# acids-ircam/RAVE

Hardware: AMD Instinct MI355X
Metric: audio samples/sec/GPU (RAVE v2 training step, 44.1 kHz, n_signal=65536) (higher is better)
Workload: dtype f32; 1 GPU; v2 config, batch 32 mono 44.1 kHz n_signal=65536, VAE-phase training step per GPU (--phase vae); global_batch=32, parallelism=dp1, phase=vae

## Files before the change

rave_amd/csrc/conv_wgrad_x6.hip:

```cpp
#include <cstdlib>
#include <mutex>
#include <type_traits>
#include "conv_params.hpp"

namespace {

typedef unsigned u32x4 __attribute__((ext_vector_type(4)));
constexpr unsigned kOOB = 0x80000000u;

struct Wx6P {
    const float* R;
    const float* S;
    float* out;
    float* rsum;
    int B, M, C, T, N;
    int r_row, s_row, s_valid, is;
    float r_slope, s_slope;
    int steps_per_b;
    int total_steps, steps_per_z;
    unsigned r_bytes, s_bytes;
    int minoff, maxoff;
    int p8, cpb, chmax;
    int av;
    unsigned b_stage;
    const unsigned* r_range;
    const unsigned* s_range;
    int off[kMaxTaps];
};

typedef u32x4 u32x4_u __attribute__((aligned(2)));

__device__ __forceinline__ void emit(const float (&v)[8], float slope, float sc, u32x4* dst, int piece_stride) {
#if RH_X6_F16
    u32x4 hi, lo;
#pragma unroll
    for (int k = 0; k < 4; ++k) {
        float a = v[2 * k] * sc, b = v[2 * k + 1] * sc;
        a = rh_max1(a, a * slope);
        b = rh_max1(b, b * slope);
        const rh_h2 h = rh_h2_split(a, b);
        hi[k] = h.hi; lo[k] = h.lo;
    }
    dst[0] = hi;
    dst[piece_stride] = lo;
#else
    unsigned h[3][8];
#pragma unroll
    for (int i = 0; i < 8; ++i) {
        const float x = rh_max1(v[i], v[i] * slope);
        rh_bf3_split(x, h[0][i], h[1][i], h[2][i]);
    }
#pragma unroll
    for (int s3 = 0; s3 < 3; ++s3) {
        u32x4 pk;
#pragma unroll
        for (int k = 0; k < 4; ++k) pk[k] = __builtin_amdgcn_perm(h[s3][2 * k + 1], h[s3][2 * k], 0x07060302u);
        dst[s3 * piece_stride] = pk;
    }
#endif
}

constexpr int kKS = 2;
constexpr int kOct = 2 * kKS;
constexpr int kSpan = 16 * kKS;

constexpr int wx6_gs(int rows) { return kX6P * rows + 4; }
constexpr int wx6_stage(int rows) { return kKS * 2 * wx6_gs(rows); }
constexpr int wx6_slot(int o, int row, int rows) { return (o >> 1) * 2 * wx6_gs(rows) + (o & 1) * wx6_gs(rows) + row; }

struct Wx6Scale { float r, s, out; };
__device__ __forceinline__ Wx6Scale wx6_scales(const Wx6P& p) {
#if RH_X6_F16
    int inv_r, inv_s;
    Wx6Scale sc;
    sc.r = __uint_as_float(rh_x6_scale_bits(rh_range_max(p.r_range), &inv_r));
    sc.s = __uint_as_float(rh_x6_scale_bits(rh_range_max(p.s_range), &inv_s));
    sc.out = __uint_as_float(rh_x6_unscale_bits(inv_r, inv_s));
    return sc;
#else
    return Wx6Scale{1.f, 1.f, 1.f};
#endif
}

struct Wx6Step {
    int n;
    unsigned rs, ss;
    bool r_tail, s_edge;
};
template <bool PL>
__device__ __forceinline__ Wx6Step wx6_step(const Wx6P& p, int st) {
    Wx6Step sp;
    const int b = st / p.steps_per_b;
    sp.n = (st - b * p.steps_per_b) * kSpan;
    sp.rs = (unsigned)((b * p.M * p.r_row + sp.n) * 4);
    sp.ss = (unsigned)((b * p.C * p.s_row + sp.n * p.is) * 4);
    sp.r_tail = sp.n + kSpan > p.r_row;
    sp.s_edge = PL ? (sp.n + p.minoff < 0 || sp.n + p.minoff + 8 * p.p8 > p.s_valid || sp.r_tail)
                   : (sp.n * p.is + p.minoff < 0 || (sp.n + kSpan - 1) * p.is + p.maxoff >= p.s_valid || sp.r_tail);
    return sp;
}

template <int NT, int BM>
struct Wx6RTasks {
    static constexpr int NA = (kOct * BM + NT - 1) / NT;
    unsigned off[NA];
    int dst[NA], pos[NA];
    float v[NA][8];
    float sum[NA];

    __device__ __forceinline__ void init(const Wx6P& p, int tid, int m0) {
#pragma unroll
        for (int q = 0; q < NA; ++q) {
            const int u = tid + NT * q;
            const int o = u % kOct, m = u / kOct;
            const bool ok = m < BM && m0 + m < p.M;
            dst[q] = m < BM ? wx6_slot(o, m, BM) : -1;
            pos[q] = 8 * o;
            off[q] = ok ? (unsigned)(((m0 + m) * p.r_row + 8 * o) * 4) : kOOB;
            sum[q] = 0.f;
#pragma unroll
            for (int i = 0; i < 8; ++i) v[q][i] = 0.f;
        }
    }
    template <class RSRC>
    __device__ __forceinline__ void load(const Wx6P& p, RSRC rsrc, const Wx6Step& sp, bool av) {
#pragma unroll
        for (int q = 0; q < NA; ++q) {
            const unsigned base = off[q] == kOOB ? kOOB : off[q] + sp.rs;
            if (av) {
#pragma unroll
                for (int h = 0; h < 2; ++h) {
                    unsigned o = base == kOOB ? kOOB : base + 16u * h;
                    if (sp.r_tail) o = sp.n + pos[q] + 4 * h < p.r_row ? o : kOOB;
                    const u32x4 x = __builtin_bit_cast(u32x4, __builtin_amdgcn_raw_buffer_load_b128(rsrc, o, 0, 0));
#pragma unroll
                    for (int i = 0; i < 4; ++i) v[q][4 * h + i] = __uint_as_float(x[i]);
                }
            } else {
#pragma unroll
                for (int i = 0; i < 8; ++i) {
                    unsigned o = base == kOOB ? kOOB : base + 4u * i;
                    if (sp.r_tail) o = sp.n + pos[q] + i < p.r_row ? o : kOOB;
                    v[q][i] = __builtin_bit_cast(float, __builtin_amdgcn_raw_buffer_load_b32(rsrc, o, 0, 0));
                }
            }
        }
    }
    __device__ __forceinline__ void add_rows() {
#pragma unroll
        for (int q = 0; q < NA; ++q)
            sum[q] += ((v[q][0] + v[q][1]) + (v[q][2] + v[q][3])) + ((v[q][4] + v[q][5]) + (v[q][6] + v[q][7]));
    }
    __device__ __forceinline__ void store_sums(const Wx6P& p, int tid, int m0, int z) const {
#pragma unroll
        for (int q = 0; q < NA; ++q) {
            float s = sum[q];
            s += __shfl_xor(s, 1, 64);
            s += __shfl_xor(s, 2, 64);
            const int u = tid + NT * q;
            const int m = u / kOct;
            if ((u % kOct) == 0 && m < BM && m0 + m < p.M) p.rsum[(long)z * p.M + m0 + m] = s;
        }
    }
    __device__ __forceinline__ void convert(const Wx6P& p, float sc, u32x4* a_stage) const {
#pragma unroll
        for (int q = 0; q < NA; ++q)
            if (dst[q] >= 0) emit(v[q], p.r_slope, sc, a_stage + dst[q], BM);
    }
};

template <int NT, int NB, int BN, bool PL>
struct Wx6STasks {
    static_assert(PL || NT * NB == kOct * BN, "the (column, octet) tasks fill NB whole rounds");
    unsigned off[NB];
    int dst[NB], p0[NB];
    float v[NB][8];
    int c_lo;
    unsigned piece;

    __device__ __forceinline__ void init(const Wx6P& p, int first, int n0, bool part) {
        c_lo = PL ? n0 / p.T : 0;
        const int n_ch = PL ? min(p.N - 1, n0 + BN - 1) / p.T - c_lo + 1 : 0;
        piece = PL ? (unsigned)(p.chmax * p.cpb) : 16u * BN;
#pragma unroll
        for (int q = 0; q < NB; ++q) {
            const int u = first + NT * q;
            if constexpr (PL) {
                const int ch = u / p.p8, o = u - ch * p.p8;
                const bool ok = ch < n_ch;
                dst[q] = ok ? ch * p.cpb + o * 16 : -1;
                p0[q] = p.minoff + 8 * o;
                off[q] = ok ? (unsigned)(((c_lo + ch) * p.s_row + p0[q]) * 4) : kOOB;
            } else {
                const int o = u % kOct, col = u / kOct;
                const int cc = (n0 + col) / p.T, t = (n0 + col) - cc * p.T;
                const bool ok = n0 + col < p.N;
                dst[q] = (ok || !part) ? wx6_slot(o, col, BN) * 16 : -1;
                p0[q] = 8 * o * p.is + (ok ? p.off[t] : 0);
                off[q] = ok ? (unsigned)((cc * p.s_row + p0[q]) * 4) : kOOB;
            }
        }
    }
    __device__ __forceinline__ unsigned column(const Wx6P& p, int n, int tn) const {
        if constexpr (PL) {
            if (n >= p.N) return 0u;
            const int cc = n / p.T, t = n - cc * p.T;
            return (unsigned)((cc - c_lo) * p.cpb + (p.off[t] - p.minoff) * 2);
        } else {
            return 16u * 32u * tn;
        }
    }
    __device__ __forceinline__ static int kblock(int kb, int g, int colj) {
        return PL ? (kb * 16 + g * 8) * 2 : (kb * 2 * wx6_gs(BN) + g * wx6_gs(BN) + colj) * 16;
    }
    template <class RSRC>
    __device__ __forceinline__ void load(const Wx6P& p, RSRC rsrc, const Wx6Step& sp, int nq) {
#pragma unroll
        for (int q = 0; q < NB; ++q) {
            if (q >= nq) continue;
            const unsigned base = off[q] == kOOB ? kOOB : off[q] + sp.ss;
#pragma unroll
            for (int i = 0; i < 8; ++i) {
                unsigned o = base == kOOB ? kOOB : base + 4u * (unsigned)(i * p.is);
                if (sp.s_edge) {
                    const int pos = sp.n * p.is + p0[q] + i * p.is;
                    o = (pos >= 0 && pos < p.s_valid) ? o : kOOB;
                }
                v[q][i] = __builtin_bit_cast(float, __builtin_amdgcn_raw_buffer_load_b32(rsrc, o, 0, 0));
            }
        }
    }
    __device__ __forceinline__ void convert(const Wx6P& p, float sc, unsigned char* b_stage, int nq) const {
#pragma unroll
        for (int q = 0; q < NB; ++q) {
            if (q >= nq || dst[q] < 0) continue;
            emit(v[q], p.s_slope, sc, reinterpret_cast<u32x4*>(b_stage + dst[q]), (int)(piece >> 4));
        }
    }
};

template <int TM, int TN, int BM, bool PL>
__device__ __forceinline__ void wx6_mma(f32x16 (&acc)[TM][TN], const u32x4* al, const unsigned char* bl, const unsigned (&bcol)[TN],
                                        unsigned piece, bool live2) {
    constexpr int SA[RH_X6_NPROD] = RH_X6_SA, SB[RH_X6_NPROD] = RH_X6_SB;
    rh_x6_frag afr[TM][kX6P], bfr[TN][kX6P];
#pragma unroll
    for (int tm = 0; tm < TM; ++tm)
#pragma unroll
        for (int s3 = 0; s3 < kX6P; ++s3) afr[tm][s3] = __builtin_bit_cast(rh_x6_frag, al[s3 * BM + tm * 32]);
#pragma unroll
    for (int tn = 0; tn < TN; ++tn)
#pragma unroll
        for (int s3 = 0; s3 < kX6P; ++s3) {
            const unsigned char* f = bl + bcol[tn] + (unsigned)s3 * piece;
            if constexpr (PL) bfr[tn][s3] = __builtin_bit_cast(rh_x6_frag, *reinterpret_cast<const u32x4_u*>(f));
            else bfr[tn][s3] = __builtin_bit_cast(rh_x6_frag, *reinterpret_cast<const u32x4*>(f));
        }
#pragma unroll
    for (int q = 0; q < RH_X6_NPROD; ++q)
#pragma unroll
        for (int tm = 0; tm < TM; ++tm) {
            acc[tm][0] = RH_X6_MFMA(afr[tm][SA[q]], bfr[0][SB[q]], acc[tm][0]);
            if constexpr (TN == 2) {
                if (live2) acc[tm][1] = RH_X6_MFMA(afr[tm][SA[q]], bfr[1][SB[q]], acc[tm][1]);
            }
        }
}

__device__ __forceinline__ void wx6_store_tile(const Wx6P& p, float* __restrict__ outz, const f32x16& acc, int mb, int col, float osc) {
#pragma unroll
    for (int r = 0; r < 16; ++r) {
        const int m = mb + (r & 3) + 8 * (r >> 2);
        if (m < p.M) outz[(long)m * p.N + col] = RH_X6_F16 ? acc[r] * osc : acc[r];
    }
}

template <int TM, int WM, int WN, bool AV, bool PART, bool PL>
__global__ __launch_bounds__(256, 2) void wgrad_x6_kernel(const Wx6P p) {
    static_assert(WM * WN == 4, "four waves");
    constexpr int NT = 256, BM = 32 * TM * WM, BN = 64 * WN;
    constexpr int NB = PL ? ((BN / 2 + 2) * 7 + NT - 1) / NT : kOct * BN / NT;
    extern __shared__ __attribute__((aligned(16))) unsigned char smem_raw[];
    u32x4* const a_st = reinterpret_cast<u32x4*>(smem_raw);
    unsigned char* const b_st = smem_raw + wx6_stage(BM) * 16;

    const int tid = threadIdx.x, lane = tid & 63;
    const int wave = __builtin_amdgcn_readfirstlane(tid >> 6);
    const int j = lane & 31, g = lane >> 5;
    const int wm = wave / WN, wn = wave - wm * WN;
    const int m0 = blockIdx.y * BM, n0 = blockIdx.x * BN, z = blockIdx.z;

    const auto r_rsrc = __builtin_amdgcn_make_buffer_rsrc(const_cast<float*>(p.R), 0, p.r_bytes, 0x00020000);
    const auto s_rsrc = __builtin_amdgcn_make_buffer_rsrc(const_cast<float*>(p.S), 0, p.s_bytes, 0x00020000);
    const Wx6Scale sc = wx6_scales(p);

    Wx6RTasks<NT, BM> rt;
    Wx6STasks<NT, NB, BN, PL> stk;
    rt.init(p, tid, m0);
    stk.init(p, tid, n0, PART);
    unsigned bcol[2];
#pragma unroll
    for (int tn = 0; tn < 2; ++tn) bcol[tn] = stk.column(p, n0 + wn * 64 + tn * 32 + j, tn);

    f32x16 acc[TM][2];
#pragma unroll
    for (int tm = 0; tm < TM; ++tm)
#pragma unroll
        for (int tn = 0; tn < 2; ++tn)
#pragma unroll
            for (int r = 0; r < 16; ++r) acc[tm][tn][r] = 0.f;

    const bool want_rsum = p.rsum != nullptr && blockIdx.x == 0;
    auto load = [&](int st) {
        const Wx6Step sp = wx6_step<PL>(p, st);
        rt.load(p, r_rsrc, sp, AV);
        stk.load(p, s_rsrc, sp, NB);
    };
    auto convert = [&]() {
        if (want_rsum) rt.add_rows();
        rt.convert(p, sc.r, a_st);
        stk.convert(p, sc.s, b_st, NB);
    };

    const int st0 = z * p.steps_per_z;
    const int nst = min(p.steps_per_z, p.total_steps - st0);
    if (nst > 0) {
        load(st0);
        convert();
    }
    __syncthreads();
    const u32x4* const al = a_st + g * wx6_gs(BM) + wm * TM * 32 + j;
    const int live_tn = !PART ? 2 : (n0 + wn * 64 >= p.N ? 0 : (n0 + wn * 64 + 32 >= p.N ? 1 : 2));
    const bool live1 = live_tn >= 1, live2 = live_tn == 2;
    for (int s = 0; s < nst; ++s) {
        const bool more = s + 1 < nst;
        if (more) load(st0 + s + 1);
        if (live1) {
#pragma unroll
            for (int kb = 0; kb < kKS; ++kb)
                wx6_mma<TM, 2, BM, PL>(acc, al + kb * 2 * wx6_gs(BM), b_st + stk.kblock(kb, g, wn * 64 + j), bcol, stk.piece, live2);
        }
        __syncthreads();
        if (more) convert();
        __syncthreads();
    }

    if (want_rsum) rt.store_sums(p, tid, m0, z);
    float* __restrict__ outz = p.out + (long)z * p.M * p.N;
#pragma unroll
    for (int tn = 0; tn < 2; ++tn) {
        const int col = n0 + wn * 64 + tn * 32 + j;
        if (col >= p.N) continue;
#pragma unroll
        for (int tm = 0; tm < TM; ++tm) wx6_store_tile(p, outz, acc[tm][tn], m0 + (wm * TM + tm) * 32 + 4 * g, col, sc.out);
    }
}

template <int NW, bool PL>
__global__ __launch_bounds__(64 * NW) void wgrad_x6_wide_kernel(const Wx6P p) {
    constexpr int TM = 3, BM = 32 * TM, BN = 32 * NW, NT = 64 * NW;
    constexpr int NB = 2;
    extern __shared__ __attribute__((aligned(16))) unsigned char smem_raw[];
    u32x4* const a_st = reinterpret_cast<u32x4*>(smem_raw);
    unsigned char* const b_st = smem_raw + 2 * wx6_stage(BM) * 16;

    const int tid = threadIdx.x, lane = tid & 63;
    const int wave = __builtin_amdgcn_readfirstlane(tid >> 6);
    const int j = lane & 31, g = lane >> 5;
    const int z = blockIdx.x;

    const auto r_rsrc = __builtin_amdgcn_make_buffer_rsrc(const_cast<float*>(p.R), 0, p.r_bytes, 0x00020000);
    const auto s_rsrc = __builtin_amdgcn_make_buffer_rsrc(const_cast<float*>(p.S), 0, p.s_bytes, 0x00020000);
    const Wx6Scale sc = wx6_scales(p);

    Wx6RTasks<NT, BM> rt;
    Wx6STasks<NT, NB, BN, PL> stk;
    rt.init(p, tid, 0);
    stk.init(p, NT - 1 - tid, 0, true);
    const int nq = PL ? (p.C * p.p8 + NT - 1) / NT : NB;
    const bool r_wave = !(NT > kOct * BM && 64 * wave >= kOct * BM);
    const int col = 32 * wave + j;
    const bool live = 32 * wave < p.N;
    const unsigned bcol[1] = {stk.column(p, col, 0)};

    f32x16 acc[TM][1];
#pragma unroll
    for (int tm = 0; tm < TM; ++tm)
#pragma unroll
        for (int r = 0; r < 16; ++r) acc[tm][0][r] = 0.f;

    const bool want_rsum = p.rsum != nullptr;
    auto load = [&](int st) {
        const Wx6Step sp = wx6_step<PL>(p, st);
        if (r_wave) rt.load(p, r_rsrc, sp, p.av != 0);
        stk.load(p, s_rsrc, sp, nq);
    };
    auto convert = [&](int stage) {
        if (want_rsum) rt.add_rows();
        rt.convert(p, sc.r, a_st + stage * wx6_stage(BM));
        stk.convert(p, sc.s, b_st + stage * p.b_stage, nq);
    };
    auto multiply = [&](int stage) {
        const u32x4* const al = a_st + stage * wx6_stage(BM) + g * wx6_gs(BM) + j;
        const unsigned char* const bs = b_st + stage * p.b_stage;
#pragma unroll
        for (int kb = 0; kb < kKS; ++kb)
            wx6_mma<TM, 1, BM, PL>(acc, al + kb * 2 * wx6_gs(BM), bs + stk.kblock(kb, g, col), bcol, stk.piece, false);
    };

    const int st0 = z * p.steps_per_z;
    const int nst = min(p.steps_per_z, p.total_steps - st0);
    if (nst > 0) {
        load(st0);
        convert(0);
    }
    __syncthreads();
    for (int s = 0; s < nst; ++s) {
        const bool more = s + 1 < nst;
        if (more) load(st0 + s + 1);
        if (live) multiply(s & 1);
        if (more) convert((s + 1) & 1);
        __syncthreads();
    }

    if (want_rsum) rt.store_sums(p, tid, 0, z);
    if (col < p.N) {
        float* __restrict__ outz = p.out + (long)z * p.M * p.N;
#pragma unroll
        for (int tm = 0; tm < TM; ++tm) wx6_store_tile(p, outz, acc[tm][0], tm * 32 + 4 * g, col, sc.out);
    }
}

struct Wx6Plan {
    int tm, wm, rt, ct, Z, steps_per_z;
    int planes;
    int nw;
    int own_z;
    size_t lds;
};

struct Wx6Env {
    bool off;
    int planes;
    int wide;
    int blocks;
    int all;
    int tm;
    bool forced_tm() const { return tm >= 1 && tm <= 3; }
};

Wx6Env read_wx6_env() {
    const auto num = [](const char* name, int dflt) { const char* e = getenv(name); return e ? atoi(e) : dflt; };
    static const int all = num("RH_WGRAD_X6_ALL", 0), tm = num("RH_WGRAD_X6_TM", 0);
    const char* pe = getenv("RH_WGRAD_X6_PLANES");
    return Wx6Env{num("RH_WGRAD_X6", 1) == 0, pe ? (pe[0] == '1' ? 1 : 0) : -1, num("RH_WGRAD_X6_WIDE", 1), num("RH_WGRAD_X6_BLOCKS", 0), all, tm};
}

bool wx6_eligible(const WgradP& w, const Wx6Env& env, const unsigned* r_range, const unsigned* s_range) {
    if (env.off) return false;
    if (RH_X6_F16 && (!r_range || !s_range)) return false;
    if (w.inner != 1 || w.T > kMaxTaps || w.B <= 0 || w.r_row <= 0) return false;
    if ((w.r_act != RH_ACT_NONE && w.r_act != RH_ACT_LEAKY) || (w.s_act != RH_ACT_NONE && w.s_act != RH_ACT_LEAKY)) return false;
    if ((w.r_act == RH_ACT_LEAKY && !(w.r_slope >= 0.f && w.r_slope <= 1.f)) || (w.s_act == RH_ACT_LEAKY && !(w.s_slope >= 0.f && w.s_slope <= 1.f))) return false;
    if (w.M < 32 || (long)w.C * w.T < 64) return false;
    if (!env.all && w.M <= 64 && w.r_row > 1024) return false;
    return 4ull * w.B * w.M * (unsigned long long)w.r_row < 0x7fffffffull && 4ull * w.B * w.C * (unsigned long long)w.s_row < 0x7fffffffull;
}

bool wx6_plane_geometry(const WgradP& w, int chmax, Wx6P* p, size_t* bytes) {
    const int reach = w.maxoff - w.minoff;
    p->p8 = (32 + reach + 7) / 8;
    p->cpb = 16 * ((p->p8 & 1) ? p->p8 : p->p8 + 1);
    p->chmax = chmax;
    *bytes = (size_t)kX6P * chmax * p->cpb + 32;
    return w.is == 1 && w.T >= 2 && reach >= 0 && p->p8 <= 7 && 4l * (w.s_row + 64) * w.C * w.B < 0x7fffffffl;
}

int wx6_choose_tile(const WgradP& w, const Wx6Env& env, Wx6P* p, Wx6Plan* pl) {
    const int Mp = (w.M + 31) & ~31;
    pl->tm = (Mp % 128 == 0 && Mp >= 256 && w.T > 1) ? 2 : (Mp % 96 == 0 ? 3 : (Mp % 64 == 0 ? 2 : 1));
    if (env.forced_tm()) pl->tm = env.tm;
    pl->wm = Mp >= 64 * pl->tm ? 2 : 1;
    const int BM = 32 * pl->tm * pl->wm, BN = 64 * (4 / pl->wm);
    pl->rt = rh_cdiv(w.M, BM);
    pl->ct = rh_cdiv(p->N, BN);
    const int four_wave_tiles = pl->rt * pl->ct;
    pl->nw = 0; pl->own_z = 0;
    size_t plane_bytes;
    if (env.wide != 0 && env.planes < 0 && !env.forced_tm() && w.M > 64 && w.M <= 96 && p->N <= 288) {
        const int tiles = rh_cdiv(p->N, 32);
        pl->nw = tiles <= 3 ? 3 : (tiles <= 4 ? 4 : (tiles <= 6 ? 6 : 9));
        pl->own_z = env.wide != 2;
        pl->tm = 3; pl->wm = 1; pl->rt = 1; pl->ct = 1;
        pl->planes = wx6_plane_geometry(w, w.C, p, &plane_bytes);
        p->av = w.r_row % 4 == 0 && ((uintptr_t)w.R & 15) == 0;
        p->b_stage = (unsigned)(pl->planes ? (plane_bytes + 15) / 16 * 16 : (size_t)wx6_stage(32 * pl->nw) * 16);
        pl->lds = 2 * ((size_t)wx6_stage(96) * 16 + p->b_stage);
    } else {
        const bool on = env.planes >= 0 ? env.planes == 1 : Mp <= 96;
        pl->planes = wx6_plane_geometry(w, BN / w.T + 2, p, &plane_bytes) && on && pl->tm >= 2;
        pl->lds = (size_t)wx6_stage(BM) * 16 + (pl->planes ? plane_bytes : (size_t)wx6_stage(BN) * 16);
    }
    return four_wave_tiles;
}

void wx6_slice_k(const Wx6Env& env, int four_wave_tiles, Wx6P* p, Wx6Plan* pl) {
    const int dflt = pl->nw == 9 && pl->own_z ? 256 : 512;
    const int target = env.blocks > 0 ? env.blocks : (env.blocks < 0 ? (pl->tm == 2 ? 768 : 512) : dflt);
    int Z = rh_cdiv(target, pl->own_z ? 1 : four_wave_tiles);
    const int zmax = p->total_steps / 4 > 0 ? p->total_steps / 4 : 1;
    if (Z > zmax) Z = zmax;
    if (Z < 1) Z = 1;
    pl->steps_per_z = rh_cdiv(p->total_steps, Z);
    pl->Z = rh_cdiv(p->total_steps, pl->steps_per_z);
    p->steps_per_z = pl->steps_per_z;
}

bool plan_wx6(const WgradP& w, Wx6P* p, Wx6Plan* pl, const unsigned* r_range, const unsigned* s_range) {
    const Wx6Env env = read_wx6_env();
    if (!wx6_eligible(w, env, r_range, s_range)) return false;
    *p = Wx6P{};
    p->R = w.R; p->S = w.S;
    p->B = w.B; p->M = w.M; p->C = w.C; p->T = w.T; p->N = w.C * w.T;
    p->r_row = w.r_row; p->s_row = w.s_row; p->s_valid = w.s_valid; p->is = w.is;
    p->r_slope = w.r_act == RH_ACT_LEAKY ? w.r_slope : 1.f;
    p->s_slope = w.s_act == RH_ACT_LEAKY ? w.s_slope : 1.f;
    p->steps_per_b = rh_cdiv(w.r_row, kSpan);
    p->total_steps = w.B * p->steps_per_b;
    p->r_bytes = (unsigned)(4ull * w.B * w.M * w.r_row); p->s_bytes = (unsigned)(4ull * w.B * w.C * w.s_row);
    p->minoff = w.minoff; p->maxoff = w.maxoff;
    p->r_range = r_range; p->s_range = s_range;
    for (int t = 0; t < w.T; ++t) p->off[t] = w.off[t];
    wx6_slice_k(env, wx6_choose_tile(w, env, p, pl), p, pl);
    return true;
}

using Wx6Launch = void (*)(dim3 grid, int threads, size_t lds, hipStream_t stream, const Wx6P& p);

template <void (*KERN)(Wx6P)>
void launch_wx6(dim3 grid, int threads, size_t lds, hipStream_t stream, const Wx6P& p) {
    static std::once_flag once;
    std::call_once(once, [] {
        (void)hipFuncSetAttribute(reinterpret_cast<const void*>(KERN), hipFuncAttributeMaxDynamicSharedMemorySize, 160 * 1024);
    });
    rh_launch_main(KERN, grid, dim3(threads), lds, stream, p);
}

template <int... Vs, class F>
Wx6Launch wx6_pick(int v, F f) {
    Wx6Launch r = nullptr;
    ((v == Vs ? (void)(r = f(std::integral_constant<int, Vs>{})) : (void)0), ...);
    return r;
}

Wx6Launch wx6_instance(const Wx6P& p, const Wx6Plan& pl) {
    if (pl.nw > 0)
        return wx6_pick<3, 4, 6, 9>(pl.nw, [&](auto NW) {
            return wx6_pick<0, 1>(pl.planes, [&](auto PL) -> Wx6Launch { return launch_wx6<wgrad_x6_wide_kernel<decltype(NW)::value, decltype(PL)::value != 0>>; });
        });
    const int av = p.r_row % 4 == 0 && ((uintptr_t)p.R & 15) == 0;
    const int part = rh_cdiv(p.N, 32) % (2 * (4 / pl.wm)) != 0;
    return wx6_pick<1, 2, 3>(pl.tm, [&](auto TM) {
        return wx6_pick<1, 2>(pl.wm, [&](auto WM) {
            return wx6_pick<0, 1>(av, [&](auto AV) {
                return wx6_pick<0, 1>(part, [&](auto PART) {
                    return wx6_pick<0, 1>(pl.planes, [&](auto PL) -> Wx6Launch {
                        constexpr int tm = decltype(TM)::value, wm = decltype(WM)::value;
                        constexpr bool planes = decltype(PL)::value != 0 && tm >= 2;
                        return launch_wx6<wgrad_x6_kernel<tm, wm, 4 / wm, decltype(AV)::value != 0, decltype(PART)::value != 0, planes>>;
                    });
                });
            });
        });
    });
}

}

int64_t rh_wgrad_x6_workspace(const WgradP& w) {
    Wx6P p;
    Wx6Plan pl{};
    static const unsigned any_range[kRangeSlotWords] = {};
    if (!plan_wx6(w, &p, &pl, any_range, any_range)) return -1;
    return (pl.Z > 1 ? (int64_t)pl.Z * w.M * w.C * w.T : 0) * (int64_t)sizeof(float) + (int64_t)pl.Z * w.M * (int64_t)sizeof(float);
}

bool rh_wgrad_x6_plan_info(const WgradP& w, int32_t* out4) {
    Wx6P p;
    Wx6Plan pl{};
    static const unsigned any_range[kRangeSlotWords] = {};
    if (!plan_wx6(w, &p, &pl, any_range, any_range)) return false;
    out4[0] = pl.nw > 0 ? pl.nw : 4;
    out4[1] = pl.rt * pl.ct * pl.Z;
    out4[2] = pl.Z;
    out4[3] = pl.planes;
    return true;
}

int rh_wgrad_x6_launch(const WgradP& w, float* dw, float* rsum_out, void* ws, hipStream_t stream, bool* used, int* left_z,
                       const unsigned* r_range, const unsigned* s_range) {
    *used = false;
    if (left_z) *left_z = 0;
    Wx6P p;
    Wx6Plan pl{};
    if (!plan_wx6(w, &p, &pl, r_range, s_range)) return RH_OK;
    p.out = pl.Z > 1 ? (float*)ws : dw;
    float* const rs_part = (float*)ws + (pl.Z > 1 ? (long)pl.Z * w.M * w.C * w.T : 0);
    p.rsum = rsum_out ? (pl.Z > 1 ? rs_part : rsum_out) : nullptr;
    const dim3 grid = pl.nw > 0 ? dim3(pl.Z) : dim3(pl.ct, pl.rt, pl.Z);
    wx6_instance(p, pl)(grid, pl.nw > 0 ? 64 * pl.nw : 256, pl.lds, stream, p);
    if (int e = rh_check_launch("conv1d_bwd_weight_x6")) return e;
    *used = true;
    if (pl.Z > 1) {
        if (left_z) *left_z = pl.Z;
        else if (int e = rh_reduce_partials_launch((const float*)ws, dw, (long)w.M * w.C * w.T, pl.Z, stream, "conv1d_bwd_weight_reduce")) return e;
        if (rsum_out) return rh_reduce_partials_launch(rs_part, rsum_out, w.M, pl.Z, stream, "conv1d_bwd_bias_reduce");
    }
    return RH_OK;
}
```

Measured before the change: 244.6 million samples/s.

## Add tall 8-wave wgrad kernel with larger M×N tiles for big conv layers

Adds a 512-thread weight-gradient kernel that uses taller tiles (4 waves along M, 2 along N, up to 4 MFMA column tiles per wave) with double-buffered LDS staging. It is selected by a heuristic for layers with large M and C*T. The K-split count is derived from a fixed block target and can be overridden through a new env var. The goal is more operand reuse per LDS load and fewer split-K partials, at the cost of higher register and LDS pressure per block and lower occupancy.

```diff
diff --git a/rave_amd/csrc/conv_wgrad_x6.hip b/rave_amd/csrc/conv_wgrad_x6.hip
--- a/rave_amd/csrc/conv_wgrad_x6.hip
+++ b/rave_amd/csrc/conv_wgrad_x6.hip
@@ -241,7 +241,7 @@
 
 template <int TM, int TN, int BM, bool PL>
 __device__ __forceinline__ void wx6_mma(f32x16 (&acc)[TM][TN], const u32x4* al, const unsigned char* bl, const unsigned (&bcol)[TN],
-                                        unsigned piece, bool live2) {
+                                        unsigned piece, int live) {
     constexpr int SA[RH_X6_NPROD] = RH_X6_SA, SB[RH_X6_NPROD] = RH_X6_SB;
     rh_x6_frag afr[TM][kX6P], bfr[TN][kX6P];
 #pragma unroll
@@ -261,9 +261,9 @@
 #pragma unroll
         for (int tm = 0; tm < TM; ++tm) {
             acc[tm][0] = RH_X6_MFMA(afr[tm][SA[q]], bfr[0][SB[q]], acc[tm][0]);
-            if constexpr (TN == 2) {
-                if (live2) acc[tm][1] = RH_X6_MFMA(afr[tm][SA[q]], bfr[1][SB[q]], acc[tm][1]);
-            }
+#pragma unroll
+            for (int tn = 1; tn < TN; ++tn)
+                if (tn < live) acc[tm][tn] = RH_X6_MFMA(afr[tm][SA[q]], bfr[tn][SB[q]], acc[tm][tn]);
         }
 }
 
@@ -331,14 +331,14 @@
     __syncthreads();
     const u32x4* const al = a_st + g * wx6_gs(BM) + wm * TM * 32 + j;
     const int live_tn = !PART ? 2 : (n0 + wn * 64 >= p.N ? 0 : (n0 + wn * 64 + 32 >= p.N ? 1 : 2));
-    const bool live1 = live_tn >= 1, live2 = live_tn == 2;
+    const bool live1 = live_tn >= 1;
     for (int s = 0; s < nst; ++s) {
         const bool more = s + 1 < nst;
         if (more) load(st0 + s + 1);
         if (live1) {
 #pragma unroll
             for (int kb = 0; kb < kKS; ++kb)
-                wx6_mma<TM, 2, BM, PL>(acc, al + kb * 2 * wx6_gs(BM), b_st + stk.kblock(kb, g, wn * 64 + j), bcol, stk.piece, live2);
+                wx6_mma<TM, 2, BM, PL>(acc, al + kb * 2 * wx6_gs(BM), b_st + stk.kblock(kb, g, wn * 64 + j), bcol, stk.piece, live_tn);
         }
         __syncthreads();
         if (more) convert();
@@ -405,7 +405,7 @@
         const unsigned char* const bs = b_st + stage * p.b_stage;
 #pragma unroll
         for (int kb = 0; kb < kKS; ++kb)
-            wx6_mma<TM, 1, BM, PL>(acc, al + kb * 2 * wx6_gs(BM), bs + stk.kblock(kb, g, col), bcol, stk.piece, false);
+            wx6_mma<TM, 1, BM, PL>(acc, al + kb * 2 * wx6_gs(BM), bs + stk.kblock(kb, g, col), bcol, stk.piece, 1);
     };
 
     const int st0 = z * p.steps_per_z;
@@ -431,11 +431,96 @@
     }
 }
 
+template <int TM, int TN>
+__global__ __launch_bounds__(512) void wgrad_x6_tall_kernel(const Wx6P p) {
+    constexpr int WN = 2, NT = 512, BM = 32 * TM * 4, BN = 32 * TN * WN;
+    constexpr int NB = kOct * BN / NT;
+    extern __shared__ __attribute__((aligned(16))) unsigned char smem_raw[];
+    u32x4* const a_st = reinterpret_cast<u32x4*>(smem_raw);
+    unsigned char* const b_st = smem_raw + 2 * wx6_stage(BM) * 16;
+    constexpr unsigned kBStage = wx6_stage(BN) * 16;
+
+    const int tid = threadIdx.x, lane = tid & 63;
+    const int wave = __builtin_amdgcn_readfirstlane(tid >> 6);
+    const int j = lane & 31, g = lane >> 5;
+    const int wm = wave / WN, wn = wave - wm * WN;
+    const int m0 = blockIdx.y * BM, n0 = blockIdx.x * BN, z = blockIdx.z;
+
+    const auto r_rsrc = __builtin_amdgcn_make_buffer_rsrc(const_cast<float*>(p.R), 0, p.r_bytes, 0x00020000);
+    const auto s_rsrc = __builtin_amdgcn_make_buffer_rsrc(const_cast<float*>(p.S), 0, p.s_bytes, 0x00020000);
+    const Wx6Scale sc = wx6_scales(p);
+
+    Wx6RTasks<NT, BM> rt;
+    Wx6STasks<NT, NB, BN, false> stk;
+    rt.init(p, tid, m0);
+    stk.init(p, tid, n0, true);
+    const int col0 = n0 + wn * 32 * TN + j;
+    unsigned bcol[TN];
+#pragma unroll
+    for (int tn = 0; tn < TN; ++tn) bcol[tn] = stk.column(p, col0 + tn * 32, tn);
+    const int live = m0 + wm * 32 * TM >= p.M ? 0 : min(TN, max(0, (p.N - (n0 + wn * 32 * TN) + 31) / 32));
+
+    f32x16 acc[TM][TN];
+#pragma unroll
+    for (int tm = 0; tm < TM; ++tm)
+#pragma unroll
+        for (int tn = 0; tn < TN; ++tn)
+#pragma unroll
+            for (int r = 0; r < 16; ++r) acc[tm][tn][r] = 0.f;
+
+    const bool want_rsum = p.rsum != nullptr && blockIdx.x == 0;
+    auto load = [&](int st) {
+        const Wx6Step sp = wx6_step<false>(p, st);
+        rt.load(p, r_rsrc, sp, p.av != 0);
+        stk.load(p, s_rsrc, sp, NB);
+    };
+    auto convert = [&](int stage) {
+        if (want_rsum) rt.add_rows();
+        rt.convert(p, sc.r, a_st + stage * wx6_stage(BM));
+        stk.convert(p, sc.s, b_st + stage * kBStage, NB);
+    };
+    auto multiply = [&](int stage) {
+        const u32x4* const al = a_st + stage * wx6_stage(BM) + g * wx6_gs(BM) + wm * TM * 32 + j;
+        const unsigned char* const bs = b_st + stage * kBStage;
+#pragma unroll
+        for (int kb = 0; kb < kKS; ++kb)
+            wx6_mma<TM, TN, BM, false>(acc, al + kb * 2 * wx6_gs(BM), bs + stk.kblock(kb, g, wn * 32 * TN + j), bcol, stk.piece, live);
+    };
+
+    const int st0 = z * p.steps_per_z;
+    const int nst = min(p.steps_per_z, p.total_steps - st0);
+    if (nst > 0) {
+        load(st0);
+        convert(0);
+    }
+    __syncthreads();
+    for (int s = 0; s < nst; ++s) {
+        const bool more = s + 1 < nst;
+        if (more) load(st0 + s + 1);
+        if (live > 0) multiply(s & 1);
+        if (more) convert((s + 1) & 1);
+        __syncthreads();
+    }
+
+    if (want_rsum) rt.store_sums(p, tid, m0, z);
+    float* __restrict__ outz = p.out + (long)z * p.M * p.N;
+#pragma unroll
+    for (int tn = 0; tn < TN; ++tn) {
+        const int col = col0 + tn * 32;
+        if (col >= p.N) continue;
+#pragma unroll
+        for (int tm = 0; tm < TM; ++tm) wx6_store_tile(p, outz, acc[tm][tn], m0 + (wm * TM + tm) * 32 + 4 * g, col, sc.out);
+    }
+}
+constexpr bool kWx6Tall = 2 * (wx6_stage(256) + wx6_stage(256)) * 16 <= 160 * 1024;
+
 struct Wx6Plan {
     int tm, wm, rt, ct, Z, steps_per_z;
     int planes;
     int nw;
     int own_z;
+    int tall;
+    int tn;
     size_t lds;
 };
 
@@ -443,7 +528,9 @@
     bool off;
     int planes;
     int wide;
+    int tall;
     int blocks;
+    int kslices;
     int all;
     int tm;
     bool forced_tm() const { return tm >= 1 && tm <= 3; }
@@ -453,7 +540,8 @@
     const auto num = [](const char* name, int dflt) { const char* e = getenv(name); return e ? atoi(e) : dflt; };
     static const int all = num("RH_WGRAD_X6_ALL", 0), tm = num("RH_WGRAD_X6_TM", 0);
     const char* pe = getenv("RH_WGRAD_X6_PLANES");
-    return Wx6Env{num("RH_WGRAD_X6", 1) == 0, pe ? (pe[0] == '1' ? 1 : 0) : -1, num("RH_WGRAD_X6_WIDE", 1), num("RH_WGRAD_X6_BLOCKS", 0), all, tm};
+    return Wx6Env{num("RH_WGRAD_X6", 1) == 0, pe ? (pe[0] == '1' ? 1 : 0) : -1, num("RH_WGRAD_X6_WIDE", 1), num("RH_WGRAD_X6_TALL", 1),
+                  num("RH_WGRAD_X6_BLOCKS", 0), num("RH_WGRAD_X6_KSLICES", 0), all, tm};
 }
 
 bool wx6_eligible(const WgradP& w, const Wx6Env& env, const unsigned* r_range, const unsigned* s_range) {
@@ -476,6 +564,11 @@
     return w.is == 1 && w.T >= 2 && reach >= 0 && p->p8 <= 7 && 4l * (w.s_row + 64) * w.C * w.B < 0x7fffffffl;
 }
 
+bool wx6_tall_wins(const WgradP& w) {
+    const long n = (long)w.C * w.T;
+    return (w.M % 256 == 0 && w.M >= 768 && n >= 2304) || (w.M == 384 && n == 384);
+}
+
 int wx6_choose_tile(const WgradP& w, const Wx6Env& env, Wx6P* p, Wx6Plan* pl) {
     const int Mp = (w.M + 31) & ~31;
     pl->tm = (Mp % 128 == 0 && Mp >= 256 && w.T > 1) ? 2 : (Mp % 96 == 0 ? 3 : (Mp % 64 == 0 ? 2 : 1));
@@ -485,9 +578,21 @@
     pl->rt = rh_cdiv(w.M, BM);
     pl->ct = rh_cdiv(p->N, BN);
     const int four_wave_tiles = pl->rt * pl->ct;
-    pl->nw = 0; pl->own_z = 0;
+    pl->nw = 0; pl->own_z = 0; pl->tall = 0; pl->tn = 2;
     size_t plane_bytes;
-    if (env.wide != 0 && env.planes < 0 && !env.forced_tm() && w.M > 64 && w.M <= 96 && p->N <= 288) {
+    if (kWx6Tall && env.tall != 0 && env.planes < 0 && !env.forced_tm() && w.M >= 256 && (env.tall == 2 || wx6_tall_wins(w))) {
+        pl->tall = 1;
+        pl->own_z = env.tall != 2;
+        pl->tm = (w.M % 384 == 0 && w.M % 256 != 0) ? 3 : 2;
+        pl->tn = pl->tm == 3 ? 2 : 4;
+        pl->wm = 4;
+        const int tall_bm = 32 * pl->tm * 4, tall_bn = 32 * pl->tn * 2;
+        pl->rt = rh_cdiv(w.M, tall_bm);
+        pl->ct = rh_cdiv(p->N, tall_bn);
+        pl->planes = 0;
+        p->av = w.r_row % 4 == 0 && ((uintptr_t)w.R & 15) == 0;
+        pl->lds = 2 * (size_t)(wx6_stage(tall_bm) + wx6_stage(tall_bn)) * 16;
+    } else if (env.wide != 0 && env.planes < 0 && !env.forced_tm() && w.M > 64 && w.M <= 96 && p->N <= 288) {
         const int tiles = rh_cdiv(p->N, 32);
         pl->nw = tiles <= 3 ? 3 : (tiles <= 4 ? 4 : (tiles <= 6 ? 6 : 9));
         pl->own_z = env.wide != 2;
@@ -507,9 +612,10 @@
 void wx6_slice_k(const Wx6Env& env, int four_wave_tiles, Wx6P* p, Wx6Plan* pl) {
     const int dflt = pl->nw == 9 && pl->own_z ? 256 : 512;
     const int target = env.blocks > 0 ? env.blocks : (env.blocks < 0 ? (pl->tm == 2 ? 768 : 512) : dflt);
-    int Z = rh_cdiv(target, pl->own_z ? 1 : four_wave_tiles);
+    int Z = pl->tall && pl->own_z ? (env.blocks > 0 ? env.blocks : 256) / (pl->rt * pl->ct) : rh_cdiv(target, pl->own_z ? 1 : four_wave_tiles);
     const int zmax = p->total_steps / 4 > 0 ? p->total_steps / 4 : 1;
     if (Z > zmax) Z = zmax;
+    if (env.kslices > 0) Z = env.kslices < p->total_steps ? env.kslices : p->total_steps;
     if (Z < 1) Z = 1;
     pl->steps_per_z = rh_cdiv(p->total_steps, Z);
     pl->Z = rh_cdiv(p->total_steps, pl->steps_per_z);
@@ -554,6 +660,9 @@
 }
 
 Wx6Launch wx6_instance(const Wx6P& p, const Wx6Plan& pl) {
+    if constexpr (kWx6Tall) {
+        if (pl.tall) return pl.tm == 3 ? launch_wx6<wgrad_x6_tall_kernel<3, 2>> : launch_wx6<wgrad_x6_tall_kernel<2, 4>>;
+    }
     if (pl.nw > 0)
         return wx6_pick<3, 4, 6, 9>(pl.nw, [&](auto NW) {
             return wx6_pick<0, 1>(pl.planes, [&](auto PL) -> Wx6Launch { return launch_wx6<wgrad_x6_wide_kernel<decltype(NW)::value, decltype(PL)::value != 0>>; });
@@ -590,7 +699,7 @@
     Wx6Plan pl{};
     static const unsigned any_range[kRangeSlotWords] = {};
     if (!plan_wx6(w, &p, &pl, any_range, any_range)) return false;
-    out4[0] = pl.nw > 0 ? pl.nw : 4;
+    out4[0] = pl.tall ? 8 : (pl.nw > 0 ? pl.nw : 4);
     out4[1] = pl.rt * pl.ct * pl.Z;
     out4[2] = pl.Z;
     out4[3] = pl.planes;
@@ -608,7 +717,7 @@
     float* const rs_part = (float*)ws + (pl.Z > 1 ? (long)pl.Z * w.M * w.C * w.T : 0);
     p.rsum = rsum_out ? (pl.Z > 1 ? rs_part : rsum_out) : nullptr;
     const dim3 grid = pl.nw > 0 ? dim3(pl.Z) : dim3(pl.ct, pl.rt, pl.Z);
-    wx6_instance(p, pl)(grid, pl.nw > 0 ? 64 * pl.nw : 256, pl.lds, stream, p);
+    wx6_instance(p, pl)(grid, pl.tall ? 512 : (pl.nw > 0 ? 64 * pl.nw : 256), pl.lds, stream, p);
     if (int e = rh_check_launch("conv1d_bwd_weight_x6")) return e;
     *used = true;
     if (pl.Z > 1) {
```

After: 240.6 million samples/s. 0.984x the previous value.
